# AlanLiangC/PDM-SSD

Hardware: AMD Instinct MI355X
Metric: frames/sec (16384-pt clouds, bs=32) (higher is better)
Workload: dtype f32; 1 GPU; configs[2]: full PDM-SSD forward (PointNet2MSG backbone + PDM neck + hybrid head: BEV heat-map head + point box head with decoded boxes), bs=32/GPU x 16384 pts, uniform KITTI-range clouds, fp32 inference, inputs resident in HBM, 4 distinct batches in rotation; launch=hipGraph, parallelism=dp1, global_batch=32

## Files before the change

### include/pdmssd_hip.h

```cpp
#ifndef PDMSSD_HIP_H
#define PDMSSD_HIP_H

#include <stddef.h>

#ifdef __cplusplus
extern "C" {
#endif

#define PDM_ABI_VERSION 1

#define PDM_E_BADARG (-1)
#define PDM_E_TOOLARGE (-2)

int pdm_abi_version(void);
const char *pdm_last_error(void);


int pdm_ball_query(void *stream, int b, int n, int m, float radius, int nsample,
                   const float *new_xyz, const float *xyz, int *idx);

int pdm_group_points(void *stream, int b, int c, int n, int npoints, int nsample,
                     const float *points, const int *idx, float *out);

int pdm_group_points_grad(void *stream, int b, int c, int n, int npoints, int nsample,
// ... 381 lines not shown
                         const int *metrics, int nC, int nD, int K, const double *overlaps, long long NP,
                         const signed char *ign_gt, long long NG, const signed char *ign_dt, long long ND,
                         const double *dt_score, const double *min_overlap, const int *slot_off, long long SV, double *slab);
int pdm_kitti_eval_pass2(void *stream, int F, const int *gt_off, const int *dt_off, const int *ov_off, int max_dt, int nM,
                         const int *metrics, int nC, int nD, int K, const double *overlaps, long long NP,
                         const signed char *ign_gt, long long NG, const signed char *ign_dt, long long ND,
                         const double *dt_score, const double *gt_alpha, const double *dt_alpha, const double *gt_bbox,
                         const double *dt_bbox, const int *gt_name, const double *min_overlap, const double *thresholds,
                         const int *num_thresholds, int compute_aos, void *workspace, size_t workspace_bytes, long long *sums);

size_t pdm_kitti_data_fov_workspace_bytes(int B);
size_t pdm_kitti_data_boxes_workspace_bytes(int B, int M);
int pdm_kitti_data_fov_count(void *stream, int B, int C, long long total_rows, const float *raw, const int *counts,
                             const float *V2C, const float *R0, const float *P2, const int *image_shape, long long capacity,
                             int *out_counts, int *overflow, unsigned char *flags, void *workspace, size_t workspace_bytes);
int pdm_kitti_data_fov_fill(void *stream, int B, int C, long long total_rows, const float *raw, const int *counts,
                            const float *V2C, const float *R0, const float *P2, const int *image_shape, long long capacity,
                            int *out_counts, int *overflow, float *out_rows, void *workspace, size_t workspace_bytes);
int pdm_kitti_data_boxes_count(void *stream, int B, int C, long long total_rows, const float *raw, const int *counts,
                               const float *V2C, const float *R0, const float *P2, const int *image_shape, int M,
                               const float *boxes, const int *box_count, int *num_points_in_gt, int *db_count,
                               long long *totals, void *workspace, size_t workspace_bytes);
int pdm_kitti_data_boxes_fill(void *stream, int B, int C, long long total_rows, const float *raw, const int *counts,
                              const float *V2C, const float *R0, const float *P2, const int *image_shape, int M,
                              const float *boxes, const int *box_count, const double *centres, int *num_points_in_gt,
                              int *db_count, long long *totals, long long capacity_points, long long capacity_entries,
                              float *out_points, long long *out_offsets, float *out_boxes, void *workspace,
                              size_t workspace_bytes);

int pdm_interp_concat_rows(void *stream, int b, int n, int m, int c2, int c1, int ld, const void *known, int known_bf16,
                           const void *skip, int skip_bf16, const int *idx, const float *weight, void *out);
int pdm_interp_concat_rows_grad(void *stream, int b, int n, int m, int c2, int ld, const void *dx, const int *idx,
                                const float *weight, float *dknown, void *workspace, size_t workspace_bytes);
int pdm_interp_concat_rows_grad_out(void *stream, int b, int n, int m, int c2, int ld, const void *dx, const int *idx,
                                    const float *weight, void *dknown, int out_bf16, void *workspace, size_t workspace_bytes);

int pdm_tg_stats_parts(long long rows, int N);
int pdm_tg_gemm_nt(void *stream, long long R, int K, int N, const void *X, long long ldx, const void *W, long long ldw,
                   void *Y, long long ldy, const float *bias, float *stats, const float *x_bn_coef);
int pdm_tg_gemm_nt_dy(void *stream, long long R, int K, int N, const void *dZ, long long lddz, const void *Yp, long long ldyp,
                      const void *W, long long ldw, void *dX, long long lddx, void *dYout, long long lddy, const float *coef,
                      const float *grads);
int pdm_tg_gemm_nt_bs(void *stream, long long R, int K, int N, const void *X, long long ldx, const void *W, long long ldw,
                      void *Y, long long ldy, const void *Bx, long long ldbx, const float *bcoef, float *bstats);
int pdm_tg_gemm_nt_pool(void *stream, long long R, int K, int N, const void *X, long long ldx, const void *W, long long ldw,
                        void *Y, long long ldy, const float *bias, float *stats, const float *x_bn_coef, int ns, void *xmax,
                        void *xmin, unsigned char *imax, unsigned char *imin);
int pdm_tg_dy_stats_parts(long long rows, int N);
int pdm_tg_gemm_nt_dy_bs(void *stream, long long R, int K, int N, const void *dZ, long long lddz, const void *Yp, long long ldyp,
                         const void *W, long long ldw, void *dX, long long lddx, void *dYout, long long lddy, const float *coef,
                         const float *grads, const void *Bx, long long ldbx, const float *bcoef, float *bstats);
size_t pdm_tg_wgrad_ws_bytes(long long R, int K, int N);
int pdm_tg_wgrad(void *stream, long long R, int K, int N, const void *dY, long long ldy, const void *X, long long ldx, float *dW,
                 int accumulate, void *workspace, size_t workspace_bytes, const float *x_bn_coef);
size_t pdm_tg_colsum_ws_floats(long long R, int N);
int pdm_tg_colsum(void *stream, long long R, int N, const void *Y, long long ld, float *out, float *scratch);
int pdm_tg_pack_weight(void *stream, int N, int K, const float *W, void *Wb, int ldb, void *Wt, int ldt);
int pdm_tg_pack_weight_pair(void *stream, int N, int K, const float *W, void *Wb, void *Wt, int rows_to, int cols_to);
int pdm_tg_pack_weight_many(void *stream, int njobs, const void *jobs, long long total_blocks);


int pdm_tune_fps_variant(int v);
int pdm_tune_fused_waves(int w);
int pdm_tune_fused_tiles(int t);
int pdm_tune_fused_groups(int n);
int pdm_tune_fused_wg_per_cu(int n);
int pdm_tune_fused_lds_cap(int bytes);
int pdm_tune_fused_reg(int on);
int pdm_tune_fused_gemm(int on);
int pdm_tune_fused_chain(int on);
int pdm_tune_fused_swz(int on);
int pdm_tune_bq_quad(int form);
int pdm_tune_bq_dense_ppc(int hundredths);
int pdm_tune_grid_split(int min_n);
int pdm_tune_bq_small_waves(int w);
int pdm_tune_bq_cpw(int centres);
int pdm_tune_bq_heavy(int candidates);
int pdm_tune_group_lds_floor(int bytes);
int pdm_tune_group_rows(int packed);
int pdm_tune_rows_chain_wg_per_cu(int n);
int pdm_tune_fp_head_tiles(int n);
int pdm_tune_rows_chain_dw_wg_per_cu(int n);
int pdm_tune_rows_chain_xcd(int on);
int pdm_tune_fp_chain_pad_lds(int bytes);
int pdm_tune_fp_chain_nt(int on);
int pdm_tune_fp_chain_mask(int m);
int pdm_tune_group_nt(int on);
int pdm_tune_copy_variant(int v);
int pdm_tune_copy_max_wg(int n);

int pdm_copy_many(void *stream, int count, void *const *dst, const void *const *src, const size_t *bytes);
int pdm_copy_many_dyn(void *stream, int count, void *const *dst, const void *const *src, const size_t *bytes,
                      const int *const *dyn_count, const unsigned *dyn_unit);


int pdm_scatter_bev(void *stream, int B, int P, int C, int degree, const float *xyz,
                    const float *feat, const float *sh, const float *inv2s2, float ox, float oy,
                    float oz, float cx, float cy, float cz, float icx, float icy, float icz, int W,
                    int H, int D, int kx, int ky, int kz, int layout, float *grid, float *wsum);

int pdm_bev_normalize(void *stream, int B, int C, int W, int H, int D, int layout, float eps,
                      float *grid, const float *wsum);

size_t pdm_gather_bev_workspace_bytes(int B, int P, int W, int H, int kx, int ky);
int pdm_gather_bev(void *stream, int B, int P, int C, int degree, const float *xyz, const float *feat,
                   const float *sh, const float *inv2s2, float ox, float oy, float oz, float cx, float cy,
                   float cz, float icx, float icy, float icz, int W, int H, int D, int kx, int ky, int kz,
                   int normalize, float eps, float *grid, float *wsum, void *workspace, size_t workspace_bytes);

int pdm_bev_normalize_grad(void *stream, int B, int C, int W, int H, int D, float eps, const float *y,
                           const float *wsum, const float *dy, float *dx, float *dwsum);

int pdm_scatter_bev_grad(void *stream, int B, int P, int C, int degree, const float *xyz,
                         const float *feat, const float *sh, const float *inv2s2, float ox,
                         float oy, float oz, float cx, float cy, float cz, float icx, float icy,
                         float icz, int W, int H, int D, int kx, int ky, int kz, int layout,
                         const float *dgrid, const float *dwsum, float *dfeat, float *dsh,
                         float *dinv2s2);
int pdm_scatter_bev_grad_normalized(void *stream, int B, int P, int C, int degree, const float *xyz,
                                    const float *feat, const float *sh, const float *inv2s2, float ox,
                                    float oy, float oz, float cx, float cy, float cz, float icx, float icy,
                                    float icz, int W, int H, int D, int kx, int ky, int kz, int layout,
                                    const float *dy, const float *wsum, float eps, const float *dwsum,
                                    float *dfeat, float *dsh, float *dinv2s2);

int pdm_topk_sampling(void *stream, int b, int n, int k, const float *scores, int *idx);

size_t pdm_pillar_assign_workspace_bytes(int N, int B, int nx, int ny);
int pdm_pillar_assign(void *stream, int N, int C1, const float *points, int B, int nx, int ny, int nz, float x0, float y0,
                      float vx, float vy, int *kept_idx, int *unq_inv, int *voxel_coords, int *pillar_count,
                      float *pillar_mean, int *cell_table, int *seg_start, int *seg_rows, int *record, void *workspace,
                      size_t workspace_bytes);
int pdm_pillar_features(void *stream, int n_kept, int C1, const float *points, const int *kept_idx, const int *unq_inv,
                        const int *voxel_coords, const float *pillar_mean, int abs_xyz, int with_dist, float vx, float vy,
                        float xoff, float yoff, float zoff, float *out);
int pdm_pillar_segment_max(void *stream, int P, int K, const float *x, const int *seg_start, const int *seg_rows, float *x_max,
                           int *arg);
int pdm_pillar_segment_max_grad(void *stream, int n_kept, int K, const float *grad_max, const int *arg, const int *unq_inv,
                                float *grad_x);
int pdm_pillar_fused_pfn(void *stream, int P, int K, int C1, const float *points, const int *kept_idx, const int *voxel_coords,
                         const float *pillar_mean, const int *seg_start, const int *seg_rows, int abs_xyz, int with_dist,
                         float vx, float vy, float xoff, float yoff, float zoff, const float *weight, const float *scale,
                         const float *shift, float *out);
int pdm_pillar_cell_table(void *stream, int P, const int *voxel_coords, int B, int nx, int ny, int nz, int *cell_table);
int pdm_pillar_scatter(void *stream, int P, int C, const float *pillar_features, const int *cell_table, int B, int nx, int ny,
                       int nz, float *canvas);
int pdm_pillar_scatter_grad(void *stream, int P, int C, const float *grad_canvas, const int *voxel_coords, int B, int nx, int ny,
                            int nz, float *grad_features);

int pdm_hard_voxel_max_points(void);
size_t pdm_hard_voxelize_workspace_bytes(int N, int B, int nx, int ny, int nz);
int pdm_hard_voxelize(void *stream, int N, int C1, const float *points, int B, int nx, int ny, int nz, float x0, float y0, float z0,
                      float vx, float vy, float vz, int T, int max_voxels, int *slot_rows, int *voxel_coords,
                      int *voxel_num_points, float *voxels, int *record, void *workspace, size_t workspace_bytes);
int pdm_hard_voxel_materialize(void *stream, int M, int T, int C1, const float *points, const int *slot_rows, float *voxels);
int pdm_hard_voxel_mean(void *stream, int M, int T, int C1, const float *points, const int *slot_rows, const int *voxel_num_points,
                        float *out);
int pdm_hard_pillar_pfn(void *stream, int M, int K, int T, int C1, const float *points, const int *slot_rows,
                        const int *voxel_num_points, const int *voxel_coords, int abs_xyz, int with_dist, float vx, float vy, float vz,
                        float xoff, float yoff, float zoff, const float *weight, const float *scale, const float *shift, float *out);

size_t pdm_anchor_targets_workspace_bytes(int B, int M, int num_sets);
int pdm_anchor_targets(void *stream, int B, int M, int cols, int A, int A_loc, int num_sets, int num_class, const float *anchors,
                       const int *set_of_slot, const int *set_of_class, const float *matched, const float *unmatched,
                       const float *gt_boxes, int norm_by_num_examples, int *box_cls_labels, float *box_reg_targets,
                       float *reg_weights, int *num_pos, void *workspace, size_t workspace_bytes);
// ... 107 lines not shown
```

### pdm_ssd_amd/csrc/rows_chain.hip

```cpp
#include "mfma_f32.h"

namespace pdm {

#ifndef DW_PIN
#define DW_PIN 1
#endif
#ifndef DW_SL
#define DW_SL 4
#endif
typedef const __attribute__((address_space(4))) f4 *cf4c;
typedef const __attribute__((address_space(1))) f4 *gf4c;

struct RowsChainArgs {
    int rows, in_stride;
    const float *in;
    const float *wpack, *bias;
    int woff[3], boff[3];
    float *out;
    int out_stride, cout, relu_last;
    int dw_H, dw_W, dw_by_xcd;
    const float *dw_w, *dw_shift;
};

constexpr int RC_THREADS = 256;
// ... 712 lines not shown
    a.hw[0] = hw_a; a.hb[0] = hb_a; a.hw[1] = hw_b; a.hb[1] = hb_b;
    int wo = 0, bo = 0;
    for (int l = 0; l < 3; ++l) {
        a.hwoff[l] = wo; a.hboff[l] = bo;
        wo += hdims[l] * hdims[l + 1];
        bo += hdims[l + 1];
    }
    a.hout[0] = out_a; a.hout_stride[0] = out_stride_a; a.hcout[0] = cout_a;
    a.hout[1] = out_b; a.hout_stride[1] = out_stride_b; a.hcout[1] = cout_b;
    a.hrelu_last = relu_last;
    const long long tiles = (rows + 63) / 64;
    const long long per8 = (tiles + 7) / 8;
    long long wgs = 8 * ((per8 + g_fph_tiles - 1) / g_fph_tiles);
    if (wgs > (1 << 20)) wgs = 1 << 20;
    const int grid = (int)wgs;
    hipLaunchKernelGGL((fp_chain_kernel<0, 8, 8, true>), dim3(grid), dim3(RC_THREADS), 0, as_stream(stream), a);
    *launched = 1;
    return check_launch("fp_head_fused");
}

static bool rc_shape_is(int nlayers, const int *dims, int k0, int k1, int k2, int k3) {
    const int want[4] = {k0, k1, k2, k3};
    const int nl = k3 ? 3 : k2 ? 2 : 1;
    if (nlayers != nl) return false;
    for (int i = 0; i <= nl; ++i)
        if (dims[i] != 16 * want[i]) return false;
    return true;
}

int rows_chain_launch(void *stream, int rows, int cin, const float *in_pm, int nlayers, const int *dims, const float *wpack,
                      const float *bias, int relu_last, float *out_pm, int out_stride, int cout, int *launched) {
    *launched = 0;
    if (rows < 8192 || cin % 16 != 0 || nlayers < 1 || nlayers > 3 || dims[0] != cin) return 0;
    RowsChainArgs a{};
    a.rows = rows; a.in_stride = cin; a.in = in_pm; a.wpack = wpack; a.bias = bias;
    int wo = 0, bo = 0;
    for (int l = 0; l < nlayers; ++l) {
        a.woff[l] = wo; a.boff[l] = bo;
        wo += dims[l] * dims[l + 1];
        bo += dims[l + 1];
    }
    a.out = out_pm; a.out_stride = out_stride; a.cout = cout; a.relu_last = relu_last;
    const long long tiles = ((long long)rows + 63) / 64;
    const int grid = (int)(tiles < 256 * g_rc_wg_per_cu ? tiles : 256 * g_rc_wg_per_cu);
#define RC_TRY(K0, K1, K2, K3)                                                                                           \
    if (rc_shape_is(nlayers, dims, K0, K1, K2, K3)) {                                                                    \
        hipLaunchKernelGGL((rows_chain_kernel<K0, K1, K2, K3>), dim3(grid), dim3(RC_THREADS), 0, as_stream(stream), a);  \
        *launched = 1;                                                                                                   \
        return check_launch("rows_mlp_fused(chain)");                                                                    \
    }
    RC_TRY(8, 16, 16, 1)
    RC_TRY(8, 4, 4, 1)
#undef RC_TRY
    return 0;
}

int rows_chain_pair_launch(void *stream, int rows, int cin, const float *in_pm, int nlayers, const int *dims, const float *wpack_a,
                           const float *bias_a, const float *wpack_b, const float *bias_b, int relu_last, float *out_a, int out_stride_a,
                           int cout_a, float *out_b, int out_stride_b, int cout_b, int *launched) {
    *launched = 0;
    if (rows < 8192 || cin % 16 != 0 || nlayers != 3 || dims[0] != cin) return 0;
    RowsChainPairArgs a{};
    a.rows = rows; a.in_stride = cin; a.in = in_pm;
    a.wpack[0] = wpack_a; a.bias[0] = bias_a; a.wpack[1] = wpack_b; a.bias[1] = bias_b;
    int wo = 0, bo = 0;
    for (int l = 0; l < nlayers; ++l) {
        a.woff[l] = wo; a.boff[l] = bo;
        wo += dims[l] * dims[l + 1];
        bo += dims[l + 1];
    }
    a.out[0] = out_a; a.out_stride[0] = out_stride_a; a.cout[0] = cout_a;
    a.out[1] = out_b; a.out_stride[1] = out_stride_b; a.cout[1] = cout_b;
    a.relu_last = relu_last;
    const long long tiles = ((long long)rows + 63) / 64;
    const int grid = (int)(tiles < 256 * g_rc_wg_per_cu ? tiles : 256 * g_rc_wg_per_cu);
    if (rc_shape_is(nlayers, dims, 8, 16, 16, 1)) {
        hipLaunchKernelGGL((rows_chain_pair_kernel<8, 16, 16, 1>), dim3(grid), dim3(RC_THREADS), 0, as_stream(stream), a);
        *launched = 1;
        return check_launch("rows_mlp_fused_pair(chain)");
    }
    return 0;
}

int rows_chain_dw_launch(void *stream, int B, int H, int W, int C, const float *map, const float *dw_w, const float *dw_shift,
                         int nlayers, const int *dims, const float *wpack, const float *bias, int relu_last, float *out_pm,
                         int out_stride, int cout, int *launched) {
    *launched = 0;
    const long long rows = (long long)B * H * W;
    if (rows < 8192 || rows >= (1ll << 31) || C % 16 != 0 || nlayers != 3 || dims[0] != C) return 0;
    RowsChainArgs a{};
    a.rows = (int)rows; a.in_stride = C; a.in = map; a.wpack = wpack; a.bias = bias;
    int wo = 0, bo = 0;
    for (int l = 0; l < nlayers; ++l) {
        a.woff[l] = wo; a.boff[l] = bo;
        wo += dims[l] * dims[l + 1];
        bo += dims[l + 1];
    }
    a.out = out_pm; a.out_stride = out_stride; a.cout = cout; a.relu_last = relu_last;
    a.dw_H = H; a.dw_W = W; a.dw_by_xcd = g_rc_dw_xcd; a.dw_w = dw_w; a.dw_shift = dw_shift;
    const long long tiles = (long long)B * ((H + 3) / 4) * ((W + 15) / 16);
    const int grid = (int)(tiles < 256 * g_rc_dw_wg_per_cu ? tiles : 256 * g_rc_dw_wg_per_cu);
    if (rc_shape_is(nlayers, dims, 8, 4, 4, 1)) {
        hipLaunchKernelGGL((rows_chain_kernel<8, 4, 4, 1, true>), dim3(grid), dim3(RC_THREADS), 0, as_stream(stream), a);
        *launched = 1;
        return check_launch("bev_head_fused");
    }
    return 0;
}

}

extern "C" int pdm_bev_head_fused(void *stream, int B, int H, int W, int C, const float *map, const float *dw_w,
                                  const float *dw_shift, int nlayers, const int *dims, const float *wpack, const float *bias,
                                  int relu_last, float *out_pm, int out_stride, int cout) {
    using namespace pdm;
    PDM_REQUIRE(B >= 0 && H > 0 && W > 0 && C > 0, PDM_E_BADARG, "bev_head_fused: bad size");
    if (B == 0) return 0;
    PDM_REQUIRE(map && dw_w && dw_shift && dims && wpack && bias && out_pm, PDM_E_BADARG, "bev_head_fused: null pointer");
    PDM_REQUIRE(cout > 0 && cout <= out_stride && out_stride % 4 == 0 &&
                    ((reinterpret_cast<uintptr_t>(map) | reinterpret_cast<uintptr_t>(dw_w) | reinterpret_cast<uintptr_t>(dw_shift) |
                      reinterpret_cast<uintptr_t>(wpack) | reinterpret_cast<uintptr_t>(bias) | reinterpret_cast<uintptr_t>(out_pm)) & 15) == 0,
                PDM_E_BADARG, "bev_head_fused: buffers must be 16-byte aligned, out_stride a multiple of 4");
    int launched = 0;
    const int rc = rows_chain_dw_launch(stream, B, H, W, C, map, dw_w, dw_shift, nlayers, dims, wpack, bias, relu_last, out_pm,
                                        out_stride, cout, &launched);
    if (rc) return rc;
    PDM_REQUIRE(launched, PDM_E_BADARG, "bev_head_fused: no instantiation for these widths");
    return 0;
}

extern "C" int pdm_fp_head_fused(void *stream, int b, int n, int m, int c_skip, const float *z_pm, int z_stride, const float *skip_pm,
                                 const int *idx, const float *weight, const int *dims, const float *wpack, const float *bias,
                                 float *out_pm, int out_stride, int cout, const int *hdims, const float *hw_a, const float *hb_a,
                                 const float *hw_b, const float *hb_b, int relu_last, float *out_a, int out_stride_a, int cout_a,
                                 float *out_b, int out_stride_b, int cout_b) {
    PDM_REQUIRE(b >= 0 && n >= 0 && m >= 1 && c_skip >= 0, PDM_E_BADARG, "fp_head_fused: bad size");
    if (b == 0 || n == 0) return 0;
    PDM_REQUIRE(z_pm && idx && weight && dims && wpack && bias && out_pm && hdims && hw_a && hb_a && hw_b && hb_b && out_a && out_b &&
                    (c_skip == 0 || skip_pm), PDM_E_BADARG, "fp_head_fused: null pointer");
    PDM_REQUIRE(out_a != out_b && cout_a > 0 && cout_b > 0 && cout_a <= 16 && cout_b <= 16 && cout_a <= out_stride_a && cout_b <= out_stride_b &&
                    out_stride_a % 4 == 0 && out_stride_b % 4 == 0 && out_stride % 4 == 0 && cout <= out_stride && z_stride % 4 == 0 && z_stride >= 128,
                PDM_E_BADARG, "fp_head_fused: strides / widths");
    PDM_REQUIRE(((reinterpret_cast<uintptr_t>(z_pm) | reinterpret_cast<uintptr_t>(wpack) | reinterpret_cast<uintptr_t>(bias) |
                  reinterpret_cast<uintptr_t>(out_pm) | reinterpret_cast<uintptr_t>(hw_a) | reinterpret_cast<uintptr_t>(hb_a) |
                  reinterpret_cast<uintptr_t>(hw_b) | reinterpret_cast<uintptr_t>(hb_b) | reinterpret_cast<uintptr_t>(out_a) |
                  reinterpret_cast<uintptr_t>(out_b)) & 15) == 0, PDM_E_BADARG, "fp_head_fused: buffers must be 16-byte aligned");
    int launched = 0;
    const int rc = pdm::fp_head_launch(stream, b, n, m, c_skip, z_pm, z_stride, skip_pm, idx, weight, dims, wpack, bias, out_pm, out_stride,
                                       cout, hdims, hw_a, hb_a, hw_b, hb_b, relu_last, out_a, out_stride_a, cout_a, out_b, out_stride_b,
                                       cout_b, &launched);
    if (rc) return rc;
    PDM_REQUIRE(launched, PDM_E_BADARG, "fp_head_fused: no instantiation for these shapes");
    return 0;
}
```

### pdm_ssd_amd/dense_heads/pdm_heatmap_head.py

```python
import os

import numpy as np
import torch
import torch.nn as nn

from ..utils import centernet_utils, loss_utils
from .point_head_template import _get
from ..fused_bn import TrainSequential


def fused_bn_enabled():
    from .. import fused_bn
    return fused_bn.ENABLED


class _Depthwise3x3CL(torch.autograd.Function):

    @staticmethod
    @torch.amp.custom_fwd(device_type="cuda", cast_inputs=torch.float32)
    def forward(ctx, x, weight, out_bf16=False):
        from .. import _native
        rows = x.permute(0, 2, 3, 1)
        if not rows.is_contiguous():
            rows = rows.contiguous()
        B, H, W, C = rows.shape
        w9 = weight.reshape(C, 9).t().contiguous()
        out = torch.empty_like(rows, dtype=torch.bfloat16) if out_bf16 else torch.empty_like(rows)
        zero = torch.zeros(C, dtype=torch.float32, device=x.device)
        _native.call("pdm_bev_depthwise3x3_t", _native.stream(x.device), B, H, W, C, rows.data_ptr(), 0,
                     w9.data_ptr(), zero.data_ptr(), out.data_ptr(), 1 if out_bf16 else 0, 0)
        ctx.save_for_backward(rows, w9)
        ctx.out_bf16 = bool(out_bf16)
        return out.permute(0, 3, 1, 2)

    @staticmethod
    @torch.amp.custom_bwd(device_type="cuda")
    def backward(ctx, g):
        from .. import _native
        rows, w9 = ctx.saved_tensors
        B, H, W, C = rows.shape
        gb = 1 if ctx.out_bf16 else 0
        gr = (g.to(torch.bfloat16) if gb else g.float()).permute(0, 2, 3, 1)
        if not gr.is_contiguous():
            gr = gr.contiguous()
        stream = _native.stream(rows.device)
        gx = gw = None
        if ctx.needs_input_grad[0]:
            gx_rows = torch.empty_like(rows)
            zero = torch.zeros(C, dtype=torch.float32, device=rows.device)
            _native.call("pdm_bev_depthwise3x3_t", stream, B, H, W, C, gr.data_ptr(), gb, w9.flip(0).contiguous().data_ptr(),
                         zero.data_ptr(), gx_rows.data_ptr(), 0, 0)
            gx = gx_rows.permute(0, 3, 1, 2)
        if ctx.needs_input_grad[1]:
            gw9 = torch.zeros((9, C), dtype=torch.float32, device=rows.device)
            _native.call("pdm_bev_depthwise3x3_wgrad_t", stream, B, H, W, C, rows.data_ptr(), gr.data_ptr(), gb, gw9.data_ptr())
            gw = gw9.t().reshape(C, 1, 3, 3)
        return gx, gw, None


class _DepthwiseConv3x3(nn.Conv2d):

    def forward(self, x):
        if x.is_cuda and x.shape[1] % 4 == 0:
            from .. import fused_bn
            bf = self.training and fused_bn.ENABLED and fused_bn.bf16_autocast() and x.shape[1] % 8 == 0 and DEPTHWISE_BF16_OUT
            return _Depthwise3x3CL.apply(x, self.weight, bool(bf))
        return super().forward(x)


DEPTHWISE_BF16_OUT = os.environ.get("PDM_DEPTHWISE_BF16_OUT", "1") == "1"


class PDMHeatmapHead(nn.Module):
    def __init__(self, model_cfg, input_channels, num_class, class_names=None, grid_size=None, point_cloud_range=None,
                 voxel_size=None, predict_boxes_when_training=False, **kwargs):
        super().__init__()
        self.model_cfg = model_cfg
        self.num_class = num_class
        self.class_names = class_names
        self.point_cloud_range = point_cloud_range
        self.voxel_size = voxel_size
        self.feature_map_stride = _get(_get(model_cfg, 'TARGET_ASSIGNER_CONFIG', {}), 'FEATURE_MAP_STRIDE', 8)
        width = _get(model_cfg, 'SHARED_CONV_CHANNEL', 64)
        layers, c = [], input_channels
        kind = _get(model_cfg, 'CONTEXT_CONV', 'separable')
        for _ in range(_get(model_cfg, 'NUM_CONTEXT_CONV', 1)):
            if kind == 'separable':
                layers += [_DepthwiseConv3x3(c, c, 3, padding=1, groups=c, bias=False), nn.BatchNorm2d(c), nn.ReLU(),
                           nn.Conv2d(c, width, 1, bias=False), nn.BatchNorm2d(width), nn.ReLU()]
            else:
                layers += [nn.Conv2d(c, width, 3, padding=1, bias=False), nn.BatchNorm2d(width), nn.ReLU()]
            c = width
        self.shared_conv = TrainSequential(*layers)
        self.hm = TrainSequential(nn.Conv2d(c, width, 1, bias=True), nn.ReLU(), nn.Conv2d(width, num_class, 1, bias=True))
        self.hm[-1].bias.data.fill_(-2.19)
        self.add_module('hm_loss_func', loss_utils.FocalLossCenterNet())
        self.forward_ret_dict = {}

    @staticmethod
    def sigmoid(x):
        return torch.clamp(x.sigmoid(), min=1e-4, max=1 - 1e-4)

    def assign_targets(self, gt_boxes, feature_map_size):
        cfg = _get(self.model_cfg, 'TARGET_ASSIGNER_CONFIG', {})
        H, W = feature_map_size
        B, M, _ = gt_boxes.shape
        vx, vy = float(self.voxel_size[0]), float(self.voxel_size[1])
        s = self.feature_map_stride
        if gt_boxes.is_cuda and gt_boxes.dtype == torch.float32 and getattr(self, 'use_fused_loss', True) and _get(cfg, 'MAX_RADIUS', 8) <= 64:
            from .. import heatmap_loss
            return heatmap_loss.heatmap_targets(gt_boxes, self.num_class, H, W, float(self.point_cloud_range[0]), float(self.point_cloud_range[1]),
                                                vx, vy, s, _get(cfg, 'GAUSSIAN_OVERLAP', 0.1), _get(cfg, 'MIN_RADIUS', 2), _get(cfg, 'MAX_RADIUS', 8))
        cx = torch.clamp((gt_boxes[..., 0] - self.point_cloud_range[0]) / vx / s, min=0, max=W - 0.5)
        cy = torch.clamp((gt_boxes[..., 1] - self.point_cloud_range[1]) / vy / s, min=0, max=H - 0.5)
        centers_int = torch.stack((cx, cy), dim=-1).int().long()
        dx, dy = gt_boxes[..., 3] / vx / s, gt_boxes[..., 4] / vy / s
        valid = (dx > 0) & (dy > 0) & (gt_boxes[..., 7] >= 1)
        safe = torch.where(valid, dx, torch.ones_like(dx)), torch.where(valid, dy, torch.ones_like(dy))
        radius = centernet_utils.gaussian_radius(safe[0], safe[1], min_overlap=_get(cfg, 'GAUSSIAN_OVERLAP', 0.1))
        radius = torch.clamp_min(radius.int(), min=_get(cfg, 'MIN_RADIUS', 2)).long()
        cls_idx = torch.stack((torch.arange(B, device=gt_boxes.device)[:, None].expand(B, M),
                               (gt_boxes[..., 7].long() - 1).clamp(min=0)), dim=-1)
        heatmap = gt_boxes.new_zeros((B, self.num_class, H, W))
        return centernet_utils.draw_gaussians(heatmap, cls_idx, centers_int, radius, valid,
                                              max_radius=_get(cfg, 'MAX_RADIUS', 8))

    def get_loss(self, tb_dict=None):
        tb_dict = {} if tb_dict is None else tb_dict
        logits, target = self.forward_ret_dict['hm_logits'], self.forward_ret_dict['heatmap']
        w = _get(_get(_get(self.model_cfg, 'LOSS_CONFIG'), 'LOSS_WEIGHTS'), 'cls_weight', 1.0)
        if (logits.is_cuda and logits.dtype in (torch.float32, torch.bfloat16) and target.dtype == torch.float32 and target.is_contiguous()
                and getattr(self, 'use_fused_loss', True) and type(self.hm_loss_func) is loss_utils.FocalLossCenterNet):
            from .. import heatmap_loss
            hm_loss = heatmap_loss.heatmap_focal_loss(logits, target, w)
        else:
            pred = self.sigmoid(logits.float())
            hm_loss = self.hm_loss_func(pred, target) * w
        tb_dict['hm_loss'] = hm_loss.detach()
        return hm_loss, tb_dict

    def _fused_logits(self, x):
        from .. import _native, fused
        mods = list(self.shared_conv)
        if (self.training or torch.is_grad_enabled() or not x.is_cuda or x.dtype != torch.float32 or len(mods) != 6
                or not isinstance(mods[0], nn.Conv2d) or mods[0].groups != mods[0].in_channels
                or not getattr(self, 'use_fused', True) or x.shape[1] % 16 != 0):
            return None
        rows = x.permute(0, 2, 3, 1)
        if not rows.is_contiguous():
            rows = rows.contiguous()
        B, H, W, C = rows.shape
        cache = self.__dict__.setdefault('_pdm_fused_cache', {})
        key = (fused._state_key(self.shared_conv), str(x.device))
# ... 40 lines not shown
```

Baseline: 7270 frames/s.

## Add warp-specialized BEV head kernel with producer depthwise and consumer MFMA waves

Adds a new fused BEV head kernel that splits each workgroup into producer waves and consumer waves. The producer waves fetch halo tiles and compute the depthwise 3x3 plus ReLU into double-buffered LDS. The consumer waves run the three-layer MFMA MLP from LDS-resident weights at raised priority. The goal is to overlap depthwise and global loads with the matrix chain instead of running them serially within the same waves. The cost is a large LDS footprint, one workgroup per CU, and a shape-specific path (C=128, 128-64-64-16) that is enabled by default and can be switched off with an env knob.

Result: faster. 7401 frames/s (median of 6 runs) (+1.8%).

```diff
diff --git a/include/pdmssd_hip.h b/include/pdmssd_hip.h
--- a/include/pdmssd_hip.h
+++ b/include/pdmssd_hip.h
@@ -487,6 +487,7 @@
 int pdm_tune_fp_head_tiles(int n);
 int pdm_tune_rows_chain_dw_wg_per_cu(int n);
 int pdm_tune_rows_chain_xcd(int on);
+int pdm_tune_bev_head_form(int form);
 int pdm_tune_fp_chain_pad_lds(int bytes);
 int pdm_tune_fp_chain_nt(int on);
 int pdm_tune_fp_chain_mask(int m);
diff --git a/pdm_ssd_amd/csrc/bev_head_roles.hip b/pdm_ssd_amd/csrc/bev_head_roles.hip
--- /dev/null
+++ b/pdm_ssd_amd/csrc/bev_head_roles.hip
@@ -0,0 +1,301 @@
+#include "mfma_f32.h"
+
+namespace pdm {
+
+#ifndef BR_DIAG
+#define BR_DIAG 0
+#endif
+#ifndef BR_PRIO
+#define BR_PRIO 1
+#endif
+
+#ifndef BR_DEPTH
+#define BR_DEPTH 1
+#endif
+
+template <int S> struct br_slot { static constexpr int value = S; };
+typedef const __attribute__((address_space(1))) f4 *br_gf4c;
+
+struct BevRolesArgs {
+    int B, H, W, by_xcd;
+    const float *map;
+    const float *dw_w, *dw_shift;
+    const float *wpack, *bias;
+    float *out;
+    int out_stride, cout, relu_last;
+};
+
+constexpr int BR_CONS = 4, BR_PROD = 8;
+constexpr int BR_THREADS = 64 * (BR_CONS + BR_PROD);
+constexpr int BR_ROW = 34;
+constexpr int BR_TILE_F4 = 64 * BR_ROW;
+constexpr int BR_W2 = 8 * 4 * 64, BR_W3 = BR_W2 + 4 * 4 * 64, BR_W_F4 = BR_W3 + 4 * 64;
+constexpr int BR_DW = BR_W_F4 + 2 * BR_TILE_F4;
+constexpr int BR_LDS_BYTES = (BR_DW + 10 * 32) * 16;
+
+template <int NKB, int NMB>
+__device__ __forceinline__ void br_layer(const f4 (&in)[NKB], f4 (&acc)[NMB], const f4 *wl, const f4 (&bias)[NMB], float floor, f4 (&an)[4],
+                                         const f4 *next, int next_stride) {
+#pragma unroll
+    for (int mb = 0; mb < NMB; ++mb) acc[mb] = bias[mb];
+    if constexpr (NMB == 1) {
+        static_assert(NKB == 4, "br_layer: the one-block layer has four k-blocks");
+        f4 a[4];
+#pragma unroll
+        for (int i = 0; i < 4; ++i) a[i] = an[i];
+#pragma unroll
+        for (int i = 0; i < 4; ++i) an[i] = next[i * next_stride];
+        __builtin_amdgcn_sched_barrier(0);
+#pragma unroll
+        for (int kb = 0; kb < 4; ++kb) acc[0] = mfma4(acc[0], a[kb], in[kb]);
+        __builtin_amdgcn_sched_barrier(0);
+    } else {
+        static_assert(NMB == 4, "br_layer: four output blocks");
+#pragma unroll
+        for (int kb = 0; kb < NKB; ++kb) {
+            f4 a[4];
+#pragma unroll
+            for (int i = 0; i < 4; ++i) a[i] = an[i];
+#pragma unroll
+            for (int i = 0; i < 4; ++i) an[i] = kb + 1 < NKB ? wl[(i * NKB + kb + 1) * 64] : next[i * next_stride];
+            __builtin_amdgcn_sched_barrier(0);
+            mfma4_grid(&acc[0], a, in[kb]);
+            __builtin_amdgcn_sched_barrier(0);
+        }
+    }
+#pragma unroll
+    for (int mb = 0; mb < NMB; ++mb) {
+        acc[mb].x = __builtin_amdgcn_fmed3f(acc[mb].x, floor, __builtin_inff());
+        acc[mb].y = __builtin_amdgcn_fmed3f(acc[mb].y, floor, __builtin_inff());
+        acc[mb].z = __builtin_amdgcn_fmed3f(acc[mb].z, floor, __builtin_inff());
+        acc[mb].w = __builtin_amdgcn_fmed3f(acc[mb].w, floor, __builtin_inff());
+    }
+}
+
+#if BR_DIAG & 1
+#define BR_STAMP(arr, i) do { __builtin_amdgcn_s_waitcnt(0xc07f); (arr)[i] = __builtin_amdgcn_s_memtime(); } while (0)
+#else
+#define BR_STAMP(arr, i)
+#endif
+
+__global__ __launch_bounds__(BR_THREADS, 1) void bev_head_roles_kernel(BevRolesArgs a) {
+    extern __shared__ __attribute__((aligned(16))) f4 br_lds[];
+    f4 *const wl = br_lds, *const tiles = br_lds + BR_W_F4;
+    const int t = threadIdx.x, lane = t & 63;
+    const int wave = __builtin_amdgcn_readfirstlane(t >> 6);
+    const bool consumer = wave < BR_CONS;
+    const int ntx = (a.W + 15) / 16, nty = (a.H + 3) / 4;
+    const long long ntiles = (long long)a.B * nty * ntx;
+    const bool by_xcd = a.by_xcd && (gridDim.x & 7) == 0;
+    const long long per_xcd = (ntiles + 7) >> 3, nsteps = by_xcd ? per_xcd * 8 : ntiles;
+    auto tile_of = [&](long long step, int &b, int &y0, int &x0) -> bool {
+        if (step >= nsteps) return false;
+        const long long tl = by_xcd ? (step & 7) * per_xcd + (step >> 3) : step;
+        if (tl >= ntiles) return false;
+        const unsigned tu = (unsigned)tl, pp = (unsigned)(ntx * nty);
+        const unsigned bb = tu / pp, rem = tu - bb * pp, ty = rem / (unsigned)ntx;
+        b = (int)bb;
+        y0 = (int)ty * 4; x0 = (int)(rem - ty * (unsigned)ntx) * 16;
+        return true;
+    };
+    long long step = blockIdx.x;
+    int cb = 0, cy0 = 0, cx0 = 0;
+    if (!tile_of(step, cb, cy0, cx0)) return;
+    const long long stride = gridDim.x;
+#if BR_DIAG & 1
+    long long ds[8] = {};
+    int nt = 0;
+    long long *const dst = reinterpret_cast<long long *>(a.out) + (size_t)blockIdx.x * 16;
+#endif
+
+    if (!consumer) {
+        const int pw = wave - BR_CONS, ppos = lane & 15, pqq = lane >> 4, pq = 4 * pw + pqq;
+        const int e_row = (lane >> 3) < 6 ? (lane >> 3) : 5, e_right = (lane >> 2) & 1, e_q = 4 * pw + (lane & 3);
+        const int e_src = 4 * (4 * (ppos >> 3) + pqq);
+        f4 hv[BR_DEPTH][6], he[BR_DEPTH];
+        unsigned hin[BR_DEPTH];
+        auto fetch = [&](f4 (&v)[6], f4 &e, unsigned &in, long long s) {
+            int b = cb, y0 = cy0, x0 = cx0;
+            (void)tile_of(s, b, y0, x0);
+            const f4 *__restrict__ img = reinterpret_cast<const f4 *>(a.map) + (size_t)b * a.H * a.W * 32;
+            in = 0;
+            const int gx = x0 + ppos, sx = gx >= a.W ? a.W - 1 : gx;
+#pragma unroll
+            for (int ry = 0; ry < 6; ++ry) {
+                const int gy = y0 - 1 + ry, sy = gy < 0 ? 0 : gy >= a.H ? a.H - 1 : gy;
+#if BR_DIAG & 4
+                v[ry] = f4{1.f, 2.f, 3.f, (float)sx};
+#else
+                v[ry] = ((br_gf4c)img)[(unsigned)((sy * a.W + sx) * 32 + pq)];
+#endif
+                in |= (unsigned)(gy >= 0 && gy < a.H && gx < a.W) << ry;
+            }
+            const int gy = y0 - 1 + e_row, ex = e_right ? x0 + 16 : x0 - 1;
+            const int sy = gy < 0 ? 0 : gy >= a.H ? a.H - 1 : gy, sxe = ex < 0 ? 0 : ex >= a.W ? a.W - 1 : ex;
+#if BR_DIAG & 4
+            e = f4{1.f, 2.f, 3.f, (float)sxe};
+#else
+            e = ((br_gf4c)img)[(unsigned)((sy * a.W + sxe) * 32 + e_q)];
+#endif
+            in |= (unsigned)(lane < 48 && gy >= 0 && gy < a.H && ex >= 0 && ex < a.W) << 6;
+        };
+#pragma unroll
+        for (int s = 0; s < BR_DEPTH; ++s) fetch(hv[s], he[s], hin[s], step + s * stride);
+        f4 *const dwl = br_lds + BR_DW;
+        if (ppos < 9) dwl[ppos * 32 + pq] = *reinterpret_cast<const f4 *>(a.dw_w + ppos * 128 + 4 * pq);
+        if (ppos == 9) dwl[9 * 32 + pq] = *reinterpret_cast<const f4 *>(a.dw_shift + 4 * pq);
+        __builtin_amdgcn_wave_barrier();
+        auto produce = [&](const f4 (&v)[6], f4 e, unsigned in, f4 *tile) {
+            const f4 zero = {0.f, 0.f, 0.f, 0.f};
+            const f4 shift = dwl[9 * 32 + pq];
+            f4 acc[4] = {shift, shift, shift, shift};
+            if (!((in >> 6) & 1)) e = zero;
+#pragma unroll
+            for (int dy = 0; dy < 3; ++dy) {
+                const f4 k0 = dwl[(dy * 3 + 0) * 32 + pq], k1 = dwl[(dy * 3 + 1) * 32 + pq], k2 = dwl[(dy * 3 + 2) * 32 + pq];
+#pragma unroll
+                for (int o = 0; o < 4; ++o) {
+                    const int ry = o + dy;
+                    const f4 c = (in >> ry) & 1 ? v[ry] : zero;
+                    f4 l, r;
+#pragma unroll
+                    for (int j = 0; j < 4; ++j) {
+                        const int ev = __builtin_amdgcn_ds_bpermute(e_src + 32 * ry, __float_as_int(e[j]));
+                        l[j] = __int_as_float(__builtin_amdgcn_update_dpp(ev, __float_as_int(c[j]), 0x111, 0xf, 0xf, false));
+                        r[j] = __int_as_float(__builtin_amdgcn_update_dpp(ev, __float_as_int(c[j]), 0x101, 0xf, 0xf, false));
+                    }
+                    acc[o] = __builtin_elementwise_fma(k0, l, acc[o]);
+                    acc[o] = __builtin_elementwise_fma(k1, c, acc[o]);
+                    acc[o] = __builtin_elementwise_fma(k2, r, acc[o]);
+                }
+                __builtin_amdgcn_sched_barrier(0);
+            }
+#pragma unroll
+            for (int o = 0; o < 4; ++o) {
+                const f4 y = f4{fmaxf(acc[o].x, 0.f), fmaxf(acc[o].y, 0.f), fmaxf(acc[o].z, 0.f), fmaxf(acc[o].w, 0.f)};
+                tile[(o * 16 + ppos) * BR_ROW + pq] = y;
+            }
+        };
+        produce(hv[0], he[0], hin[0], tiles);
+        fetch(hv[0], he[0], hin[0], step + BR_DEPTH * stride);
+        __syncthreads();
+        int buf = 0;
+        auto iter = [&](auto slot) -> bool {
+            constexpr int s = decltype(slot)::value;
+            BR_STAMP(ds, 0);
+            int nb, ny0, nx0;
+            const bool have_next = tile_of(step + stride, nb, ny0, nx0);
+            if (have_next) produce(hv[s], he[s], hin[s], tiles + (buf ^ 1) * BR_TILE_F4);
+            BR_STAMP(ds, 1);
+            fetch(hv[s], he[s], hin[s], step + (1 + BR_DEPTH) * stride);
+            BR_STAMP(ds, 2);
+            __syncthreads();
+#if BR_DIAG & 1
+            BR_STAMP(ds, 3);
+            if (++nt == 3 && t == 64 * BR_CONS)
+                for (int i = 0; i < 4; ++i) dst[8 + i] = ds[i];
+#endif
+            step += stride;
+            buf ^= 1;
+            return have_next;
+        };
+        static_assert(BR_DEPTH >= 1 && BR_DEPTH <= 4, "bev_head_roles: halo slots");
+        for (;;) {
+            if (!iter(br_slot<1 % BR_DEPTH>{})) return;
+            if constexpr (BR_DEPTH > 1) { if (!iter(br_slot<2 % BR_DEPTH>{})) return; }
+            if constexpr (BR_DEPTH > 2) { if (!iter(br_slot<3 % BR_DEPTH>{})) return; }
+            if constexpr (BR_DEPTH > 3) { if (!iter(br_slot<0>{})) return; }
+        }
+    } else {
+#if BR_PRIO
+        __builtin_amdgcn_s_setprio(1);
+#endif
+        const int pos = lane & 15, g = lane >> 4;
+        {
+            const f4 *__restrict__ wsrc = reinterpret_cast<const f4 *>(a.wpack);
+            for (int i = t; i < BR_W_F4; i += 64 * BR_CONS) wl[i] = *(br_gf4c)(wsrc + i);
+        }
+        f4 b1[4], b2[4], b3[1];
+#pragma unroll
+        for (int mb = 0; mb < 4; ++mb) {
+            b1[mb] = *reinterpret_cast<const f4 *>(a.bias + 16 * mb + 4 * g);
+            b2[mb] = *reinterpret_cast<const f4 *>(a.bias + 64 + 16 * mb + 4 * g);
+        }
+        b3[0] = *reinterpret_cast<const f4 *>(a.bias + 128 + 4 * g);
+        const float last_floor = a.relu_last ? 0.0f : -__builtin_inff();
+        __syncthreads();
+        const f4 *const w1 = wl + lane, *const w2 = wl + BR_W2 + lane, *const w3 = wl + BR_W3 + lane;
+        f4 an[4];
+#pragma unroll
+        for (int i = 0; i < 4; ++i) an[i] = w1[i * 8 * 64];
+        int buf = 0;
+        for (;;) {
+            BR_STAMP(ds, 0);
+            const f4 *tile = tiles + buf * BR_TILE_F4 + (wave * 16 + pos) * BR_ROW + g;
+            f4 x0[8], x1[4], x2[4], x3[1];
+#pragma unroll
+            for (int kb = 0; kb < 8; ++kb) x0[kb] = tile[4 * kb];
+            BR_STAMP(ds, 1);
+            br_layer<8, 4>(x0, x1, w1, b1, 0.0f, an, w2, 4 * 64);
+            BR_STAMP(ds, 2);
+            br_layer<4, 4>(x1, x2, w2, b2, 0.0f, an, w3, 64);
+            BR_STAMP(ds, 3);
+            br_layer<4, 1>(x2, x3, w3, b3, last_floor, an, w1, 8 * 64);
+            BR_STAMP(ds, 4);
+            const bool live = cy0 + wave < a.H && cx0 + pos < a.W;
+#if !(BR_DIAG & 1)
+            if (live) {
+                const long long row = ((long long)cb * a.H + cy0 + wave) * a.W + cx0 + pos;
+                store_quad_ragged(a.out + (size_t)row * a.out_stride, 4 * g, a.cout, x3[0]);
+            }
+#else
+            asm volatile("" :: "v"(x3[0]), "v"((int)live));
+#endif
+            BR_STAMP(ds, 5);
+            int nb = 0, ny0 = 0, nx0 = 0;
+            const bool have_next = tile_of(step + stride, nb, ny0, nx0);
+            __syncthreads();
+#if BR_DIAG & 1
+            BR_STAMP(ds, 6);
+            if (++nt == 3 && t == 0)
+                for (int i = 0; i < 7; ++i) dst[i] = ds[i];
+#endif
+            if (!have_next) break;
+            step += stride;
+            cb = nb; cy0 = ny0; cx0 = nx0;
+            buf ^= 1;
+        }
+    }
+}
+
+static int g_bev_head_form = 1;
+
+int bev_head_roles_launch(void *stream, int B, int H, int W, int C, const float *map, const float *dw_w, const float *dw_shift,
+                          int nlayers, const int *dims, const float *wpack, const float *bias, int relu_last, float *out_pm,
+                          int out_stride, int cout, int grid_cap, int by_xcd, int *launched) {
+    *launched = 0;
+    if (g_bev_head_form != 1) return 0;
+    const long long rows = (long long)B * H * W;
+    if (rows < 8192 || rows >= (1ll << 31) || C != 128 || nlayers != 3 || dims[0] != 128 || dims[1] != 64 || dims[2] != 64 || dims[3] != 16 ||
+        cout > 16 || (long long)H * W * 512 >= (1ll << 31))
+        return 0;
+    BevRolesArgs a{};
+    a.B = B; a.H = H; a.W = W; a.by_xcd = by_xcd;
+    a.map = map; a.dw_w = dw_w; a.dw_shift = dw_shift; a.wpack = wpack; a.bias = bias;
+    a.out = out_pm; a.out_stride = out_stride; a.cout = cout; a.relu_last = relu_last;
+    const long long tiles = (long long)B * ((H + 3) / 4) * ((W + 15) / 16);
+    const int grid = (int)(tiles < 256 * grid_cap ? tiles : 256 * grid_cap);
+    const int rc = grant_lds(reinterpret_cast<const void *>(&bev_head_roles_kernel), BR_LDS_BYTES);
+    if (rc) { set_error("bev_head_fused: %d bytes of LDS refused (%d)", BR_LDS_BYTES, rc); return rc; }
+    hipLaunchKernelGGL(bev_head_roles_kernel, dim3(grid), dim3(BR_THREADS), BR_LDS_BYTES, as_stream(stream), a);
+    *launched = 1;
+    return check_launch("bev_head_fused(roles)");
+}
+
+}
+
+extern "C" int pdm_tune_bev_head_form(int form) {
+    const int old = pdm::g_bev_head_form;
+    if (form == 0 || form == 1) pdm::g_bev_head_form = form;
+    return old;
+}
diff --git a/pdm_ssd_amd/csrc/rows_chain.hip b/pdm_ssd_amd/csrc/rows_chain.hip
--- a/pdm_ssd_amd/csrc/rows_chain.hip
+++ b/pdm_ssd_amd/csrc/rows_chain.hip
@@ -818,6 +818,10 @@
     return 0;
 }
 
+int bev_head_roles_launch(void *stream, int B, int H, int W, int C, const float *map, const float *dw_w, const float *dw_shift,
+                          int nlayers, const int *dims, const float *wpack, const float *bias, int relu_last, float *out_pm,
+                          int out_stride, int cout, int grid_cap, int by_xcd, int *launched);
+
 int rows_chain_dw_launch(void *stream, int B, int H, int W, int C, const float *map, const float *dw_w, const float *dw_shift,
                          int nlayers, const int *dims, const float *wpack, const float *bias, int relu_last, float *out_pm,
                          int out_stride, int cout, int *launched) {
@@ -836,6 +840,9 @@
     a.dw_H = H; a.dw_W = W; a.dw_by_xcd = g_rc_dw_xcd; a.dw_w = dw_w; a.dw_shift = dw_shift;
     const long long tiles = (long long)B * ((H + 3) / 4) * ((W + 15) / 16);
     const int grid = (int)(tiles < 256 * g_rc_dw_wg_per_cu ? tiles : 256 * g_rc_dw_wg_per_cu);
+    const int rrc = bev_head_roles_launch(stream, B, H, W, C, map, dw_w, dw_shift, nlayers, dims, wpack, bias, relu_last, out_pm, out_stride,
+                                          cout, g_rc_dw_wg_per_cu, g_rc_dw_xcd, launched);
+    if (rrc || *launched) return rrc;
     if (rc_shape_is(nlayers, dims, 8, 4, 4, 1)) {
         hipLaunchKernelGGL((rows_chain_kernel<8, 4, 4, 1, true>), dim3(grid), dim3(RC_THREADS), 0, as_stream(stream), a);
         *launched = 1;
diff --git a/pdm_ssd_amd/dense_heads/pdm_heatmap_head.py b/pdm_ssd_amd/dense_heads/pdm_heatmap_head.py
--- a/pdm_ssd_amd/dense_heads/pdm_heatmap_head.py
+++ b/pdm_ssd_amd/dense_heads/pdm_heatmap_head.py
@@ -69,6 +69,9 @@
 
 
 DEPTHWISE_BF16_OUT = os.environ.get("PDM_DEPTHWISE_BF16_OUT", "1") == "1"
+if "PDM_BEV_HEAD_FORM" in os.environ:
+    from .. import _native as _native_for_form
+    _native_for_form.lib().pdm_tune_bev_head_form(int(os.environ["PDM_BEV_HEAD_FORM"]))
 
 
 class PDMHeatmapHead(nn.Module):
```
